# alan-turing-institute/mogp-emulator

Measured on AMD Instinct MI355X. Metric: GP fits/sec (+ fit+grad/s, predict pts/s), 64-output n=2000 d=10 on 1 MI355X, fp64, higher is better.
Workload: dtype f64

## Files before the change

mogp_emulator_amd/csrc/kernels_chol.hip:

```cpp
#include <algorithm>
#include <cstdlib>
#include "launch.h"
#include "chol128_dev.h"

namespace mogp {

typedef double v2d __attribute__((ext_vector_type(2)));
typedef double v4d __attribute__((ext_vector_type(4)));

__device__ __forceinline__ int slot_emu(const int* idx, int z) { return idx ? idx[z] : z; }

template <int RM>
__device__ __forceinline__ void logdet_gram_dev(const BatchView& v, int emu, double* __restrict__ res, double* red) {
  const int ld = v.LD, R = v.R;
  const double* A = v.A + (size_t)emu * v.MS;
  double s = 0.;
  double acc[RM * (RM + 1) / 2];
#pragma unroll
  for (int e = 0; e < RM * (RM + 1) / 2; ++e) acc[e] = 0.;
  for (int i = threadIdx.x; i < v.n; i += 256) {
    s += log(A[(size_t)i * ld + i]);
    double y[RM];
#pragma unroll
    for (int r = 0; r < RM; ++r) y[r] = (r < R) ? A[(size_t)(v.n + r) * ld + i] : 0.0;
// ... 225 lines not shown
      s += part[1][lane];
      s += part[2][lane];
      w[2 * lane] -= s[0];
      w[2 * lane + 1] -= s[1];
    }
    __syncthreads();
  };
  double Lc[64], rdgw = 0.0;
  const int myblk = rg == 0 ? 1 : 0;
  auto preload_diag = [&]() {
    if (rg < 2) {
      const double* Lb = Ld[myblk];
      const double dg = Lb[lane * 65 + lane];
      rdgw = (j0 + 64 * myblk + lane < n) ? 1.0 / dg : 0.0;
#pragma unroll
      for (int j = 0; j < 64; ++j) Lc[j] = Lb[j * 65 + lane];
      __builtin_amdgcn_sched_barrier(0);
#pragma unroll
      for (int j = 0; j < 64; ++j) Lc[j] *= -rdgw;
    }
  };
  auto solve_diag = [&](int blk) {
    const int k0 = j0 + 64 * blk;
    if (rg == (blk ? 0 : 1)) {
      if (!HOIST) preload_diag();
      double bs = w[64 * blk + lane] * rdgw;
      __builtin_amdgcn_sched_barrier(0);
      int xlo = 0, xhi = 0;
#pragma unroll
      for (int j = 63; j >= 0; --j) {
        const int lo = __builtin_amdgcn_readlane(__double2loint(bs), j), hi = __builtin_amdgcn_readlane(__double2hiint(bs), j);
        asm("v_writelane_b32 %0, %1, %2" : "+v"(xlo) : "s"(lo), "n"(j));
        asm("v_writelane_b32 %0, %1, %2" : "+v"(xhi) : "s"(hi), "n"(j));
        bs = __builtin_fma(Lc[j], __hiloint2double(hi, lo), bs);
      }
      double xout = __hiloint2double(xhi, xlo);
      xs[64 * blk + lane] = xout;
      if (__double_as_longlong(xout) == -1ll) xout = __builtin_nan("");
      st_agent(alpha + k0 + lane, xout);
    }
    __syncthreads();
  };
  auto poll_values = [&](int cc, int lo) {
    if (t >= lo && t < lo + 64) {
      const double* p = alpha + 128 * cc + t;
      double x = ld_agent(p);
      int spins = 0;
      while (__double_as_longlong(x) == -1ll && spins++ < spin_limit) {
        __builtin_amdgcn_s_sleep(1);
        x = ld_agent(p);
      }
      if (__double_as_longlong(x) == -1ll) {
        timed_out = 1;
        __hip_atomic_store(status + emu, epoch, __ATOMIC_RELAXED, __HIP_MEMORY_SCOPE_AGENT);
        __builtin_amdgcn_fence(__ATOMIC_RELEASE, "agent");
        x = 0.0;
      }
      xs[t] = x;
    }
    __syncthreads();
  };
  __syncthreads();
  if (HOIST) preload_diag();
  if (res && c == 0) logdet_gram_dev<1>(v, emu, res, red);
  if (nch - 1 > c) {
    load_tile(tA, 128 * (nch - 1) + 64);
    load_tile(tB, 128 * (nch - 1));
  } else {
    load_tile(tA, j0 + 64);
  }
  for (int cc = nch - 1; cc > c; --cc) {
    poll_values(cc, 64);
    apply_tile(tA, 64, 128);
    if (cc - 1 > c) load_tile(tA, 128 * (cc - 1) + 64);
    else load_tile(tA, j0 + 64);
    poll_values(cc, 0);
    apply_tile(tB, 0, 128);
    if (cc - 1 > c) load_tile(tB, 128 * (cc - 1));
  }
  solve_diag(1);
  apply_tile(tA, 64, 64);
  solve_diag(0);
  if (res && c == 0 && t == 0) {
    const int st = info[emu];
    const bool gave_up = timed_out || __hip_atomic_load(status + emu, __ATOMIC_RELAXED, __HIP_MEMORY_SCOPE_AGENT) == epoch;
    int rep = (st == 0 && gave_up) ? BACKSOLVE_TIMEOUT : st;
    if (mc_abort && *mc_abort != 0u) rep = MCHOL_ABORTED;
    res[(size_t)emu * RES_STRIDE + 1] = (double)rep;
  }
}

__global__ __launch_bounds__(256) void combine_rows_kernel(BatchView v, const double* __restrict__ M) {
  const int emu = slot_emu(v.idx, blockIdx.y);
  const int ld = v.LD, R = v.R;
  const int i = blockIdx.x * 256 + threadIdx.x;
  if (i >= ld) return;
  const double* Zb = v.Z + (size_t)emu * R * ld;
  const double* Mb = M + (size_t)emu * (RMAX + 1) * RMAX;
  double z[RMAX];
#pragma unroll
  for (int r = 0; r < RMAX; ++r) z[r] = (r < R) ? Zb[(size_t)r * ld + i] : 0.0;
  for (int c = 0; c < v.RA; ++c) {
    double s = 0.;
#pragma unroll
    for (int r = 0; r < RMAX; ++r) s = __builtin_fma(Mb[c * RMAX + r], z[r], s);
    v.alpha[((size_t)emu * v.RA + c) * ld + i] = s;
  }
}

__global__ __launch_bounds__(256) void alpha_linv_kernel(BatchView v) {
  __shared__ double red[4][128];
  typedef double a2 __attribute__((ext_vector_type(2)));
  const int emu = slot_emu(v.idx, blockIdx.y);
  const int ld = v.LD, n = v.n, R = v.R;
  const double* Li = v.Linv + (size_t)emu * v.MS;
  const int lane = threadIdx.x & 63, wave = threadIdx.x >> 6;
  const int i0 = blockIdx.x * 128, i = i0 + 2 * lane;
  for (int r = 0; r < R; ++r) {
    const double* y = v.A + (size_t)emu * v.MS + (size_t)(n + r) * ld;
    a2 s = {0., 0.};
    if (i0 < n) {
#pragma unroll 16
      for (int k = i0 + wave; k < n; k += 4) {
        const a2 l = *reinterpret_cast<const a2*>(Li + (size_t)k * ld + i);
        const double yk = y[k];
        s[0] = __builtin_fma(l[0], yk, s[0]);
        s[1] = __builtin_fma(l[1], yk, s[1]);
      }
    }
    red[wave][2 * lane] = s[0];
    red[wave][2 * lane + 1] = s[1];
    __syncthreads();
    if (threadIdx.x < 128) {
      const int c = i0 + (int)threadIdx.x, t = threadIdx.x;
      v.Z[((size_t)emu * R + r) * ld + c] = (c < n) ? red[0][t] + red[1][t] + red[2][t] + red[3][t] : 0.0;
    }
    __syncthreads();
  }
}

__global__ __launch_bounds__(256) void loo_variance_kernel(BatchView v, double* __restrict__ out, int out_ld) {
  __shared__ double red[4][64];
  const int emu = slot_emu(v.idx, blockIdx.y);
  const int ld = v.LD, n = v.n;
  const double* Li = v.Linv + (size_t)emu * v.MS;
  const int lane = threadIdx.x & 63, wave = threadIdx.x >> 6;
  const int i0 = blockIdx.x * 64, i = i0 + lane;
  double s = 0.;
#pragma unroll 8
  for (int k = i0 + wave; k < n; k += 4) {
    const double x = Li[(size_t)k * ld + i];
    s = __builtin_fma(x, x, s);
  }
  red[wave][lane] = s;
  __syncthreads();
  if (wave == 0 && i < n) out[(size_t)blockIdx.y * out_ld + i] = fmax(1.0 / (red[0][lane] + red[1][lane] + red[2][lane] + red[3][lane]), 0.0);
}

constexpr int IMPL_MAXRANK = 16;
__global__ __launch_bounds__(256) void implausibility_kernel(int nb, const double* __restrict__ mean, const double* __restrict__ var, int ld,
                                                             int m, const double* __restrict__ prm, int rank, double* __restrict__ out) {
  const int j = blockIdx.x * 256 + threadIdx.x;
  if (j >= m) return;
  double top[IMPL_MAXRANK];
#pragma unroll
  for (int r = 0; r < IMPL_MAXRANK; ++r) top[r] = -1.0;
  for (int k = 0; k < nb; ++k) {
    const double mu = mean[(size_t)k * ld + j] + prm[3 * k + 2];
    const double vv = fmax(var[(size_t)k * ld + j], 0.0) + prm[3 * k + 1];
    double I = fabs(prm[3 * k] - mu) / sqrt(vv);
#pragma unroll
    for (int r = 0; r < IMPL_MAXRANK; ++r)
      if (r <= rank && I > top[r]) {
        const double t = top[r];
        top[r] = I;
        I = t;
      }
  }
  double res = top[0];
#pragma unroll
  for (int r = 1; r < IMPL_MAXRANK; ++r)
    if (r == rank) res = top[r];
  out[j] = res;
}

__global__ __launch_bounds__(256) void implausibility_top_kernel(int nb, const double* __restrict__ mean, const double* __restrict__ var, int ld,
                                                                 int m, const double* __restrict__ prm, int keep, double* __restrict__ out,
                                                                 long out_ld) {
  const int j = blockIdx.x * 256 + threadIdx.x;
  if (j >= m) return;
  double top[IMPL_MAXRANK];
#pragma unroll
  for (int r = 0; r < IMPL_MAXRANK; ++r) top[r] = -INFINITY;
  for (int k = 0; k < nb; ++k) {
    const double mu = mean[(size_t)k * ld + j] + prm[3 * k + 2];
    const double vv = fmax(var[(size_t)k * ld + j], 0.0) + prm[3 * k + 1];
    double I = fabs(prm[3 * k] - mu) / sqrt(vv);
#pragma unroll
    for (int r = 0; r < IMPL_MAXRANK; ++r)
      if (r < keep && I > top[r]) {
        const double t = top[r];
        top[r] = I;
        I = t;
      }
  }
#pragma unroll
  for (int r = 0; r < IMPL_MAXRANK; ++r)
    if (r < keep) out[(size_t)r * out_ld + j] = top[r];
}

__global__ __launch_bounds__(256) void implausibility_merge_kernel(int nparts, const double* __restrict__ lists, long ld, int m, int rank,
                                                                  double* __restrict__ out) {
  const int j = blockIdx.x * 256 + threadIdx.x;
  if (j >= m) return;
  double top[IMPL_MAXRANK];
#pragma unroll
  for (int r = 0; r < IMPL_MAXRANK; ++r) top[r] = -1.0;
  const int keep = rank + 1;
  for (int p = 0; p < nparts; ++p)
    for (int q = 0; q < keep; ++q) {
      double I = lists[((size_t)p * keep + q) * ld + j];
#pragma unroll
      for (int r = 0; r < IMPL_MAXRANK; ++r)
        if (r <= rank && I > top[r]) {
          const double t = top[r];
          top[r] = I;
          I = t;
        }
    }
  double res = top[0];
#pragma unroll
  for (int r = 1; r < IMPL_MAXRANK; ++r)
    if (r == rank) res = top[r];
  out[j] = res;
}

constexpr int MEAN_MAXQ = RMAX;
__device__ __forceinline__ double add_nc(double a, double b) {
#pragma clang fp contract(off)
  return a + b;
}
__device__ __forceinline__ double sub_nc(double a, double b) {
#pragma clang fp contract(off)
  return a - b;
}
__device__ __forceinline__ double mul_nc(double a, double b) {
#pragma clang fp contract(off)
  return a * b;
}
__global__ __launch_bounds__(256) void predict_mean_finish_kernel(int nb, int m, int D, int R, int nbasis, const double* __restrict__ basis,
                                                                  const double* __restrict__ coef, const double* __restrict__ dots,
                                                                  const double* __restrict__ LA, double* __restrict__ mean,
                                                                  double* __restrict__ var, long ld, int nterm,
                                                                  const double* __restrict__ dbasis, const int* __restrict__ ddims,
                                                                  const int* __restrict__ dpowers, double* __restrict__ deriv) {
  const int j = blockIdx.x * 256 + threadIdx.x;
  const int k = blockIdx.y;
  if (j >= m) return;
  const double* c = coef + (size_t)k * nbasis;
  if (mean) {
    if (R == 1) {
      double v = c[0];
      for (int t = 1; t < nbasis; ++t) v = add_nc(v, mul_nc(c[t], basis[(size_t)t * m + j]));
      mean[(size_t)k * ld + j] = add_nc(mean[(size_t)k * ld + j], v);
    } else {
      const int q = R - 1;
      const double* dk = dots + (size_t)k * R * m;
      double mu = dk[j];
      for (int t = 0; t < q; ++t) mu = add_nc(mu, mul_nc(c[t], basis[(size_t)t * m + j]));
      mean[(size_t)k * ld + j] = mu;
      if (var) {
        const double* La = LA + (size_t)k * q * q;
        double rm[MEAN_MAXQ], add = 0.;
#pragma unroll
        for (int t = 0; t < MEAN_MAXQ; ++t) {
          if (t < q) {
            double sres = sub_nc(basis[(size_t)t * m + j], dk[(size_t)(1 + t) * m + j]);
#pragma unroll
            for (int p = 0; p < MEAN_MAXQ; ++p)
              if (p < t) sres = sub_nc(sres, mul_nc(La[t * q + p], rm[p]));
            rm[t] = sres / La[t * q + t];
            add = add_nc(add, mul_nc(rm[t], rm[t]));
          }
        }
        var[(size_t)k * ld + j] = add_nc(var[(size_t)k * ld + j], add);
      }
    }
  }
  if (deriv && nterm > 0) {
    for (int t = 0; t < nterm; ++t) {
      const int d = ddims[t];
      bool first = true;
      for (int u = 0; u < t; ++u) first = first && (ddims[u] != d);
      if (!first) continue;
      double mid = 0.;
      for (int u = t; u < nterm; ++u)
        if (ddims[u] == d) mid = add_nc(mid, mul_nc(mul_nc(c[u + 1], (double)dpowers[u]), dbasis[(size_t)u * m + j]));
      double* o = deriv + ((size_t)k * m + j) * D + d;
      *o = add_nc(*o, mid);
    }
  }
}

__global__ __launch_bounds__(64) void trtri_leaf_kernel(BatchView v, const double* __restrict__ Lmat) {
  __shared__ double Ls[64 * 65];
  const int emu = __builtin_amdgcn_readfirstlane(slot_emu(v.idx, blockIdx.y));
  const int ld = v.LD;
  const int d0 = blockIdx.x * 64;
  const double* __restrict__ L = Lmat + (size_t)emu * v.MS + (size_t)d0 * ld + d0;
  double* Li = v.Linv + (size_t)emu * v.MS;
  const int t = threadIdx.x;
#pragma unroll 8
  for (int r = 0; r < 64; ++r) Ls[r * 65 + t] = L[(size_t)r * ld + t];
  __builtin_amdgcn_wave_barrier();
  double x[64];
#pragma unroll
  for (int c = 0; c < 64; ++c) {
    double s0 = (c == t) ? 1.0 : 0.0, s1 = 0., s2 = 0., s3 = 0.;
#pragma unroll
    for (int p = 0; p < c; ++p) {
      const double lv = Ls[c * 65 + p];
      if ((p & 3) == 0) s0 = __builtin_fma(-x[p], lv, s0);
      else if ((p & 3) == 1) s1 = __builtin_fma(-x[p], lv, s1);
      else if ((p & 3) == 2) s2 = __builtin_fma(-x[p], lv, s2);
      else s3 = __builtin_fma(-x[p], lv, s3);
    }
    x[c] = ((s0 + s1) + (s2 + s3)) / Ls[c * 65 + c];
  }
#pragma unroll
  for (int i = 0; i < 64; ++i) Li[(size_t)(d0 + i) * ld + d0 + t] = x[i];
  if ((blockIdx.x & 1) == 0 && d0 + 64 < ld) {
#pragma unroll 8
    for (int i = 0; i < 64; ++i) Li[(size_t)(d0 + i) * ld + d0 + 64 + t] = 0.0;
  }
}

__global__ void extract_kernel(const double* __restrict__ src, int NP, int n, double* __restrict__ out, int mode) {
  const int j = blockIdx.x * blockDim.x + threadIdx.x;
  const int i = blockIdx.y;
  if (j >= n) return;
  double x;
  if (mode == 0) x = src[(size_t)i * NP + j];
  else if (mode == 1) x = (i <= j) ? src[(size_t)j * NP + i] : 0.0;
  else x = (j <= i) ? src[(size_t)i * NP + j] : src[(size_t)j * NP + i];
  out[(size_t)i * n + j] = x;
}

void launch_logdet(const BatchView& v, const int* info, double* res, hipStream_t s, const int* bs_status, int bs_epoch, const unsigned* mc_abort) {
  hipLaunchKernelGGL(logdet_kernel, dim3(v.nb), dim3(256), 0, s, v, info, res, bs_status, bs_epoch, mc_abort);
}

void launch_combine_rows(const BatchView& v, const double* M, hipStream_t s) {
  hipLaunchKernelGGL(combine_rows_kernel, dim3((v.LD + 255) / 256, v.nb), dim3(256), 0, s, v, M);
}

bool launch_backsolve_chain(const BatchView& v, int epoch, int* status, int n_cu, hipStream_t s, const int* info, double* res, const unsigned* mc_abort) {
  const int nch = (v.n + 127) / 128;
  static const int spin_limit = [] { const char* e = getenv("MOGP_BS_SPIN"); return e ? atoi(e) : (1 << 20); }();
  prof_begin("backsolve", s);
  const bool bound = v.nb * nch <= n_cu;
  double* r = (v.R == 1 && bound) ? res : nullptr;
  if (bound) hipLaunchKernelGGL(backsolve_chain_kernel<true>, dim3(v.nb * nch), dim3(256), 0, s, v, nullptr, epoch, nch, status, spin_limit, info, r, mc_abort);
  else hipLaunchKernelGGL(backsolve_chain_kernel<false>, dim3(v.nb * nch), dim3(256), 0, s, v, nullptr, epoch, nch, status, spin_limit, info, r, mc_abort);
  prof_end("backsolve", s, 0., (double)v.nb * 4.0 * (double)v.n * (double)v.n);
  return r != nullptr;
}

void launch_backsolve(const BatchView& v, hipStream_t s) {
  hipLaunchKernelGGL(backsolve_init_kernel, dim3((v.NP + 255) / 256, v.nb), dim3(256), 0, s, v);
  const int nblk = (v.n + 63) / 64;
  for (int kb = nblk - 1; kb >= 0; --kb) {
    const int k0 = kb * 64;
    const bool fused = v.R == 1;
    if (!fused || kb == nblk - 1) hipLaunchKernelGGL(backsolve_diag_kernel, dim3(v.nb), dim3(64), 0, s, v, k0);
    if (k0 > 0) {
      const dim3 grid((k0 / 2 + BSG_THREADS - 1) / BSG_THREADS, v.nb);
      if (fused) hipLaunchKernelGGL(backsolve_gemv4_kernel<true>, grid, dim3(256), 0, s, v, k0);
      else hipLaunchKernelGGL(backsolve_gemv_kernel<RMAX>, grid, dim3(BSG_THREADS), 0, s, v, k0);
    }
  }
}

void launch_alpha_from_linv(const BatchView& v, hipStream_t s) {
  hipLaunchKernelGGL(alpha_linv_kernel, dim3(v.NP / 128, v.nb), dim3(256), 0, s, v);
}

void launch_loo_variance(const BatchView& v, double* out, int out_ld, hipStream_t s) {
  hipLaunchKernelGGL(loo_variance_kernel, dim3((v.n + 63) / 64, v.nb), dim3(256), 0, s, v, out, out_ld);
}

void launch_implausibility(int nb, const double* mean, const double* var, int ld, int m, const double* prm, int rank, double* out,
                           hipStream_t s) {
  hipLaunchKernelGGL(implausibility_kernel, dim3((m + 255) / 256), dim3(256), 0, s, nb, mean, var, ld, m, prm, rank, out);
}

void launch_implausibility_top(int nb, const double* mean, const double* var, int ld, int m, const double* prm, int keep, double* out,
                               long out_ld, hipStream_t s) {
  hipLaunchKernelGGL(implausibility_top_kernel, dim3((m + 255) / 256), dim3(256), 0, s, nb, mean, var, ld, m, prm, keep, out, out_ld);
}

void launch_implausibility_merge(int nparts, const double* lists, long ld, int m, int rank, double* out, hipStream_t s) {
  hipLaunchKernelGGL(implausibility_merge_kernel, dim3((m + 255) / 256), dim3(256), 0, s, nparts, lists, ld, m, rank, out);
}

__device__ __forceinline__ double int_pow(double x, int p) {
  if (p == 0) return 1.0;
  if (p == 1) return x;
  if (p == 2) return x * x;
  return pow(x, (double)p);
}
__global__ __launch_bounds__(256) void mean_basis_kernel(const double* __restrict__ Xs, int m, int D, int nterm, const int* __restrict__ dims,
                                                         const int* __restrict__ powers, double* __restrict__ basis, double* __restrict__ dbasis) {
  const int j = blockIdx.x * 256 + threadIdx.x;
  if (j >= m) return;
  basis[j] = 1.0;
  for (int t = 0; t < nterm; ++t) {
    const double x = Xs[(size_t)j * D + dims[t]];
    basis[(size_t)(t + 1) * m + j] = int_pow(x, powers[t]);
    dbasis[(size_t)t * m + j] = int_pow(x, powers[t] - 1);
  }
}
void launch_mean_basis(const double* Xs, int m, int D, int nterm, const int* dims, const int* powers, double* basis, double* dbasis, hipStream_t s) {
  hipLaunchKernelGGL(mean_basis_kernel, dim3((m + 255) / 256), dim3(256), 0, s, Xs, m, D, nterm, dims, powers, basis, dbasis);
}

void launch_predict_mean_finish(int nb, int m, int D, int R, int nbasis, const double* basis, const double* coef, const double* dots,
                                const double* LA, double* mean, double* var, long ld, int nterm, const double* dbasis, const int* ddims,
                                const int* dpowers, double* deriv, hipStream_t s) {
  hipLaunchKernelGGL(predict_mean_finish_kernel, dim3((m + 255) / 256, nb), dim3(256), 0, s, nb, m, D, R, nbasis, basis, coef, dots, LA,
                     mean, var, ld, nterm, dbasis, ddims, dpowers, deriv);
}

void launch_trtri_merges(const BatchView& v, hipStream_t s);

void launch_trtri(const BatchView& v, hipStream_t s) {
  hipLaunchKernelGGL(trtri_leaf_kernel, dim3(v.NP / 64, v.nb), dim3(64), 0, s, v, (const double*)v.A);
  launch_trtri_merges(v, s);
}

void launch_extract(const double* src, int NP, int n, double* out, int mode, hipStream_t s) {
  hipLaunchKernelGGL(extract_kernel, dim3((n + 255) / 256, n), dim3(256), 0, s, src, NP, n, out, mode);
}

}
```

mogp_emulator_amd/csrc/kernels_gemm.hip:

```cpp
#include <algorithm>
#include <type_traits>
#include "launch.h"
#include "trsm_dev.h"
#include "gemm_dev.h"
#include "gemm_loop_dev.h"

namespace mogp {



template <int WT>
__global__ __launch_bounds__(256, 2) void update_kernel(BatchView v, int c0, int k0, int k1, int nt, int ntiles) {
  extern __shared__ __attribute__((aligned(16))) double smem[];
  using C = Cfg<WT>;
  int z, tile;
  decode_block(v.nb, ntiles, z, tile);
  if (z >= v.nb) return;
  int ti, tj;
  if (ntiles == nt) {
    ti = tile;
    tj = 0;
  } else {
    ti = (tile + 1) >> 1;
    tj = (tile > 0 && (tile & 1) == 0) ? 1 : 0;
  }
  const int emu = slot_to_emu(v.idx, z);
  double* A = v.A + (size_t)emu * v.MS;
  const int ld = v.LD;
  const int i0 = c0 + ti * C::BM, j0 = c0 + tj * C::BM;
  v4d acc[WT][WT];
  gemm_mainloop<WT, true, true>(A + (size_t)i0 * ld + k0, ld, A + (size_t)j0 * ld + k0, ld, (k1 - k0) / BK, acc, smem);
  for_each_acc<WT>(acc, [&](int r, int c, double x) {
    double* p = A + (size_t)(i0 + r) * ld + (j0 + c);
    *p -= x;
  });
}

__global__ __launch_bounds__(256, 3) void trsm128_lds_kernel(BatchView v, int c0, int r0, const double* __restrict__ Lpack128) {
  extern __shared__ __attribute__((aligned(16))) double smem[];
  const int emu = slot_to_emu(v.idx, blockIdx.y);
  trsm128_lds_dev(v, c0, r0, Lpack128 + (size_t)emu * PACK128_STRIDE, emu, blockIdx.x, smem);
}

template <int WT, int MODE>
__device__ __forceinline__ void merge_mainloop(const double* __restrict__ Ag, int lda, const double* __restrict__ Bg, int ldb, int nk, int nk_full,
                                               v4d (&acc)[WT][WT], double* smem, int wr, int wc) {
  using C = Cfg<WT>;
  const int lane = threadIdx.x & 63;
  const int fr = lane & 15, fk = lane >> 4;
#pragma unroll
  for (int i = 0; i < WT; ++i)
#pragma unroll
    for (int j = 0; j < WT; ++j) acc[i][j] = (v4d){0., 0., 0., 0.};
  if (nk <= 0) return;
  const size_t stepB = (size_t)BK * ldb;
  v2d ra[C::CH], rb[C::CH];
  const unsigned offA = g2r_off<WT, true>(lda), offB = g2r_off<WT, false>(ldb);
  g2r<WT, true>(Ag, lda, offA, ra);
  g2r<WT, false>(Bg, ldb, offB, rb);
  r2s<WT, true>(smem, ra);
  r2s<WT, false>(smem + C::OPSZ, rb);
  __syncthreads();
  auto step = [&](int kt, auto S_, auto E_) {
    constexpr int S = decltype(S_)::value, E = decltype(E_)::value;
    const double* sA = smem + (kt & 1) * 2 * C::OPSZ;
    const double* sB = sA + C::OPSZ;
    const bool more = (kt + 1 < nk);
    if (more) {
      Ag += BK;
      Bg += stepB;
      g2r<WT, true>(Ag, lda, offA, ra);
      g2r<WT, false>(Bg, ldb, offB, rb);
    }
    if (S < WT && E > 0) {
#pragma unroll
      for (int kk = 0; kk < 4; ++kk) {
        double a[WT], b[WT];
        const int k = kk * 4 + fk;
#pragma unroll
        for (int i = S; i < WT; ++i) a[i] = sA[((2 * i + wr) * 16 + fr) * LDK + k];
#pragma unroll
        for (int j = 0; j < E; ++j) b[j] = sB[k * C::LDM + (2 * j + wc) * 16 + fr];
#pragma unroll
        for (int i = S; i < WT; ++i)
#pragma unroll
          for (int j = 0; j < E; ++j) acc[i][j] = __builtin_amdgcn_mfma_f64_16x16x4f64(a[i], b[j], acc[i][j], 0, 0, 0);
      }
    }
    if (more) {
      double* dA = smem + ((kt + 1) & 1) * 2 * C::OPSZ;
      r2s<WT, true>(dA, ra);
      r2s<WT, false>(dA + C::OPSZ, rb);
    }
    __syncthreads();
  };
  using I0 = std::integral_constant<int, 0>;
  using IW = std::integral_constant<int, WT>;
  int kt = 0;
  static_assert(WT == 2 || WT == 4, "phase lists are written for two or four sub-tiles per wave");
  if (MODE == 0) {
    for (const int end = min(nk, wc); kt < end; ++kt) step(kt, I0(), I0());
    for (const int end = min(nk, 2 + wc); kt < end; ++kt) step(kt, I0(), std::integral_constant<int, 1>());
    if (WT == 4) {
      for (const int end = min(nk, 4 + wc); kt < end; ++kt) step(kt, I0(), std::integral_constant<int, 2>());
      for (const int end = min(nk, 6 + wc); kt < end; ++kt) step(kt, I0(), std::integral_constant<int, 3>());
    }
    for (; kt < nk; ++kt) step(kt, I0(), IW());
  } else {
    for (const int end = min(nk, nk_full + wr + 1); kt < end; ++kt) step(kt, I0(), IW());
    for (const int end = min(nk, nk_full + 2 + wr + 1); kt < end; ++kt) step(kt, std::integral_constant<int, 1>(), IW());
    if (WT == 4) {
      for (const int end = min(nk, nk_full + 4 + wr + 1); kt < end; ++kt) step(kt, std::integral_constant<int, 2>(), IW());
      for (const int end = min(nk, nk_full + 6 + wr + 1); kt < end; ++kt) step(kt, std::integral_constant<int, 3>(), IW());
    }
    for (; kt < nk; ++kt) step(kt, IW(), IW());
  }
}

template <int WT, int STEP>
__global__ __launch_bounds__(256, 2) void trtri_merge_kernel(BatchView v, int h, int tiles_per_dim, int nodes) {
  extern __shared__ __attribute__((aligned(16))) double smem[];
  using C = Cfg<WT>;
  const int tpn = tiles_per_dim * tiles_per_dim;
  int z, t;
  decode_block(v.nb, nodes * tpn, z, t);
  if (z >= v.nb) return;
  const int node = t / tpn, bx = t % tpn;
  const int emu = slot_to_emu(v.idx, z);
  const int ld = v.LD;
  const int base = node * 2 * h;
  if (base + h >= v.NP) return;
  const int m2 = min(h, v.NP - base - h);
  int ti, tj;
  if (STEP == 0) {
    tj = bx / tiles_per_dim;
    ti = bx % tiles_per_dim;
  } else {
    ti = tiles_per_dim - 1 - (bx / tiles_per_dim);
    tj = bx % tiles_per_dim;
  }
  const int i0 = ti * C::BM, j0 = tj * C::BM;
  if (i0 >= m2) return;
  const double* L = v.A + (size_t)emu * v.MS;
  double* Li = v.Linv + (size_t)emu * v.MS;
  double* S = v.Kinv + (size_t)emu * v.MS;
  const int lane = threadIdx.x & 63, wave = __builtin_amdgcn_readfirstlane(threadIdx.x >> 6);
  const int wr = wave >> 1, wc = wave & 1;
  v4d acc[WT][WT];
  auto store = [&](double* dst, double sign) {
#pragma unroll
    for (int i = 0; i < WT; ++i)
#pragma unroll
      for (int j = 0; j < WT; ++j)
#pragma unroll
        for (int r = 0; r < 4; ++r)
          dst[(size_t)((2 * i + wr) * 16 + (lane >> 4) + 4 * r) * ld + (2 * j + wc) * 16 + (lane & 15)] = sign * acc[i][j][r];
  };
  if (STEP == 0) {
    const double* Ag = L + (size_t)(base + h + i0) * ld + base + j0;
    const double* Bg = Li + (size_t)(base + j0) * ld + base + j0;
    merge_mainloop<WT, 0>(Ag, ld, Bg, ld, (h - j0) / BK, 0, acc, smem, wr, wc);
    store(S + (size_t)(base + h + i0) * ld + base + j0, 1.0);
  } else {
    const double* Ag = Li + (size_t)(base + h + i0) * ld + base + h;
    const double* Bg = S + (size_t)(base + h) * ld + base + j0;
    const int kend = min(i0 + C::BM, m2);
    merge_mainloop<WT, 1>(Ag, ld, Bg, ld, kend / BK, i0 / BK, acc, smem, wr, wc);
    store(Li + (size_t)(base + h + i0) * ld + base + j0, -1.0);
  }
}

template <int WT, int TRI>
__device__ __forceinline__ void kinv_mainloop(const double* __restrict__ Ag, const double* __restrict__ Bg, int ld, int nk, v4d (&acc)[WT][WT],
                                              double* smem, int wr, int wc) {
  using C = Cfg<WT>;
  const int lane = threadIdx.x & 63;
  const int fr = lane & 15, fk = lane >> 4;
  const size_t stepA = (size_t)BK * ld;
  v2d ra[C::CH], rb[C::CH];
  const unsigned offA = g2r_off<WT, false>(ld);
  g2r<WT, false>(Ag, ld, offA, ra);
  g2r<WT, false>(Bg, ld, offA, rb);
  r2s<WT, false>(smem, ra);
  r2s<WT, false>(smem + C::OPSZ, rb);
  __syncthreads();
  auto step = [&](int kt, auto E_) {
    constexpr int E = decltype(E_)::value;
    const double* sA = smem + (kt & 1) * 2 * C::OPSZ;
    const double* sB = sA + C::OPSZ;
    const bool more = (kt + 1 < nk);
    if (more) {
      Ag += stepA;
      Bg += stepA;
      g2r<WT, false>(Ag, ld, offA, ra);
      g2r<WT, false>(Bg, ld, offA, rb);
    }
    constexpr int JN = (TRI == 0) ? WT : ((TRI == 1) ? E : E - 1);
    if (E > 0 && JN > 0) {
#pragma unroll
      for (int kk = 0; kk < 4; ++kk) {
        double a[WT], b[WT];
        const int k = kk * 4 + fk;
#pragma unroll
        for (int i = 0; i < E; ++i) a[i] = sA[k * C::LDM + (2 * i + wr) * 16 + fr];
#pragma unroll
        for (int j = 0; j < JN; ++j) b[j] = sB[k * C::LDM + (2 * j + wc) * 16 + fr];
#pragma unroll
        for (int i = 0; i < E; ++i)
#pragma unroll
          for (int j = 0; j < JN; ++j)
            if (TRI == 0 || (TRI == 1 && j <= i) || (TRI == 2 && j < i)) acc[i][j] = __builtin_amdgcn_mfma_f64_16x16x4f64(a[i], b[j], acc[i][j], 0, 0, 0);
      }
    }
    if (more) {
      double* dA = smem + ((kt + 1) & 1) * 2 * C::OPSZ;
      r2s<WT, false>(dA, ra);
      r2s<WT, false>(dA + C::OPSZ, rb);
    }
    __syncthreads();
  };
  static_assert(WT == 2 || WT == 4, "phase list written for two or four sub-tiles per wave");
  int kt = 0;
  for (const int end = min(nk, wr); kt < end; ++kt) step(kt, std::integral_constant<int, 0>());
  for (const int end = min(nk, 2 + wr); kt < end; ++kt) step(kt, std::integral_constant<int, 1>());
  if (WT == 4) {
    for (const int end = min(nk, 4 + wr); kt < end; ++kt) step(kt, std::integral_constant<int, 2>());
    for (const int end = min(nk, 6 + wr); kt < end; ++kt) step(kt, std::integral_constant<int, 3>());
  }
  for (; kt < nk; ++kt) step(kt, std::integral_constant<int, WT>());
}

template <int WT>
__global__ __launch_bounds__(256, 2) void kinv_kernel(BatchView v, int ntiles, int kend) {
  extern __shared__ __attribute__((aligned(16))) double smem[];
  using C = Cfg<WT>;
  int z, tile;
  decode_block(v.nb, ntiles, z, tile);
  if (z >= v.nb) return;
  int ti = (int)((sqrt(8.0 * tile + 1.0) - 1.0) * 0.5);
  while (ti * (ti + 1) / 2 > tile) --ti;
  while ((ti + 1) * (ti + 2) / 2 <= tile) ++ti;
  const int tj = tile - ti * (ti + 1) / 2;
  const int emu = slot_to_emu(v.idx, z);
  const int ld = v.LD;
  const double* Li = v.Linv + (size_t)emu * v.MS;
  double* Ki = v.Kinv + (size_t)emu * v.MS;
  const int i0 = ti * C::BM, j0 = tj * C::BM;
  const int lane = threadIdx.x & 63, wave = __builtin_amdgcn_readfirstlane(threadIdx.x >> 6);
  const int wr = wave >> 1, wc = wave & 1;
  v4d acc[WT][WT];
#pragma unroll
  for (int i = 0; i < WT; ++i)
#pragma unroll
    for (int j = 0; j < WT; ++j) acc[i][j] = (v4d){0., 0., 0., 0.};
  const double* Ag = Li + (size_t)i0 * ld + i0;
  const double* Bg = Li + (size_t)i0 * ld + j0;
  const int nk = (kend - i0) / BK;
  if (nk <= 0) return;
  const int tri = (ti != tj) ? 0 : (wr < wc ? 2 : 1);
  if (tri == 0) kinv_mainloop<WT, 0>(Ag, Bg, ld, nk, acc, smem, wr, wc);
  else if (tri == 1) kinv_mainloop<WT, 1>(Ag, Bg, ld, nk, acc, smem, wr, wc);
  else kinv_mainloop<WT, 2>(Ag, Bg, ld, nk, acc, smem, wr, wc);
#pragma unroll
  for (int i = 0; i < WT; ++i)
#pragma unroll
    for (int j = 0; j < WT; ++j) {
      if (tri == 0 || (tri == 1 && j <= i) || (tri == 2 && j < i)) {
#pragma unroll
        for (int r = 0; r < 4; ++r)
          Ki[(size_t)(i0 + (2 * i + wr) * 16 + (lane >> 4) + 4 * r) * ld + j0 + (2 * j + wc) * 16 + (lane & 15)] = acc[i][j][r];
      }
    }
}

__global__ __launch_bounds__(256, 2) void predict_v_store_kernel(BatchView v, const double* __restrict__ Ks, int MP, int nti, int ntj,
                                                               double* __restrict__ Vout) {
  extern __shared__ __attribute__((aligned(16))) double smem[];
  using C = Cfg<4>;
  const int npairs = (nti + 1) / 2;
  const int nsr = (npairs + 3) / 4, nsc = (ntj + 15) / 16;
  int z, tile;
  decode_block(v.nb, nsr * nsc * 64, z, tile);
  if (z >= v.nb) return;
  const int st = tile >> 6, w = tile & 63;
  const int pr = (st / nsc) * 4 + (w >> 4), tj = (st % nsc) * 16 + (w & 15);
  if (pr >= npairs || tj >= ntj) return;
  const int emu = slot_to_emu(v.idx, z);
  const int ld = v.LD;
  const double* Li = v.Linv + (size_t)emu * v.MS;
  const double* K = Ks + (size_t)z * MP * ld;
  const int j0 = tj * C::BM;
  const int ti_long = nti - 1 - pr, ti_short = pr;
  double* V = Vout + (size_t)z * v.NP * MP;
  for (int pass = 0; pass < 2; ++pass) {
    if (pass == 1 && ti_short == ti_long) break;
    const int ti = pass == 0 ? ti_long : ti_short;
    const int i0 = ti * C::BM;
    v4d acc[4][4];
    gemm_mainloop<4, true, true>(Li + (size_t)i0 * ld, ld, K + (size_t)j0 * ld, ld, (i0 + C::BM) / BK, acc, smem);
    for_each_acc<4>(acc, [&](int r, int c, double x) { V[(size_t)(i0 + r) * MP + j0 + c] = x; });
  }
}

__global__ __launch_bounds__(512, 4) void update_tri8_kernel(BatchView v, int c0, int k0, int k1, int ntiles) {
  extern __shared__ __attribute__((aligned(16))) double smem[];
  using C = WCfg<128, 128, 2, 4>;
  int z, tile;
  decode_block(v.nb, ntiles, z, tile);
  if (z >= v.nb) return;
  int ti = (int)((sqrt(8.0 * tile + 1.0) - 1.0) * 0.5);
  while (ti * (ti + 1) / 2 > tile) --ti;
  while ((ti + 1) * (ti + 2) / 2 <= tile) ++ti;
  const int tj = tile - ti * (ti + 1) / 2;
  const int emu = slot_to_emu(v.idx, z);
  double* A = v.A + (size_t)emu * v.MS;
  const int ld = v.LD;
  const int i0 = c0 + ti * 128, j0 = c0 + tj * 128;
  v4d acc[C::TI][C::TJ];
  mainloop_w<128, 128, 2, 4>(A + (size_t)i0 * ld + k0, ld, A + (size_t)j0 * ld + k0, ld, (k1 - k0) / BK, acc, smem);
  for_each_acc_w<4>(acc, [&](int r, int c, double x) {
    double* p = A + (size_t)(i0 + r) * ld + (j0 + c);
    *p -= x;
  });
}

constexpr bool PV_SWZ = true;
constexpr int PVW_LGC = 3, PVW_SC = 1 << PVW_LGC, PVW_SR = 64 >> PVW_LGC;
template <int WR, int WC, bool TRI>
__global__ __launch_bounds__(64 * WR * WC, (WR * WC >= 8 ? 4 : 2)) void predict_var_w_kernel(
    BatchView v, const double* __restrict__ Ks, int MP, int nti, int ntj, double* __restrict__ partial) {
  extern __shared__ __attribute__((aligned(16))) double smem[];
  using C = WCfg<128, 128, WR, WC>;
  const int npairs = (nti + 1) / 2;
  constexpr int lgc = PVW_LGC, SC = PVW_SC, SR = PVW_SR;
  const int nsr = (npairs + SR - 1) / SR, nsc = (ntj + SC - 1) / SC;
  const int t = threadIdx.x, lane = t & 63, wave = TRI ? __builtin_amdgcn_readfirstlane(t >> 6) : (t >> 6);
  const int wr = wave / WC, wc = wave % WC;
  int z, tile;
  decode_block(v.nb, nsr * nsc * 64, z, tile);
  if (z >= v.nb) return;
  const int st = tile >> 6, w = tile & 63;
  const int pr = (st / nsc) * SR + (w >> lgc), tj = (st % nsc) * SC + (w & (SC - 1));
  if (pr >= npairs || tj >= ntj) return;
  const int emu = slot_to_emu(v.idx, z);
  const int ld = v.LD;
  const double* Li = v.Linv + (size_t)emu * v.MS;
  const double* K = Ks + (size_t)z * MP * ld;
  const int j0 = tj * 128;
  const int ti_long = nti - 1 - pr, ti_short = pr;
  for (int pass = 0; pass < 2; ++pass) {
    if (pass == 1 && ti_short == ti_long) break;
    const int ti = pass == 0 ? ti_long : ti_short;
    const int i0 = ti * 128;
    v4d acc[C::TI][C::TJ];
    const int nk = TRI ? min(i0 + 128, (v.n + 15) & ~15) / BK : (i0 + 128) / BK;
    mainloop_w<128, 128, WR, WC, TRI, true, PV_SWZ>(Li + (size_t)i0 * ld, ld, K + (size_t)j0 * ld, ld, nk, acc, smem, i0 / BK, v.n - i0);
    double* red = smem;
#pragma unroll
    for (int j = 0; j < C::TJ; ++j) {
      double s = 0.;
#pragma unroll
      for (int i = 0; i < C::TI; ++i)
#pragma unroll
        for (int r = 0; r < 4; ++r) s += acc[i][j][r] * acc[i][j][r];
      s += __shfl_xor(s, 16);
      s += __shfl_xor(s, 32);
      if (lane < 16) red[wr * 128 + wc * 16 * C::TJ + j * 16 + lane] = s;
    }
    __syncthreads();
    if (t < 128) {
      double s = 0.;
#pragma unroll
      for (int q = 0; q < WR; ++q) s += red[q * 128 + t];
      partial[((size_t)z * nti + ti) * MP + j0 + t] = s;
    }
    __syncthreads();
  }
}

__global__ __launch_bounds__(256, 2) void fullcov_kernel(BatchView v, const double* __restrict__ V, int MP, int m, int ntiles, int kend,
                                                       double* __restrict__ cov) {
  extern __shared__ __attribute__((aligned(16))) double smem[];
  using C = Cfg<4>;
  int z, tile;
  decode_block(v.nb, ntiles, z, tile);
  if (z >= v.nb) return;
  int ti = (int)((sqrt(8.0 * tile + 1.0) - 1.0) * 0.5);
  while (ti * (ti + 1) / 2 > tile) --ti;
  while ((ti + 1) * (ti + 2) / 2 <= tile) ++ti;
  const int tj = tile - ti * (ti + 1) / 2;
  const double* Vz = V + (size_t)z * v.NP * MP;
  double* Cz = cov + (size_t)z * m * m;
  const int i0 = ti * C::BM, j0 = tj * C::BM;
  v4d acc[4][4];
  gemm_mainloop<4, false, false>(Vz + i0, MP, Vz + j0, MP, kend / BK, acc, smem);
  for_each_acc<4>(acc, [&](int r, int c, double x) {
    const int i = i0 + r, j = j0 + c;
    if (i < m && j < m) {
      const double val = Cz[(size_t)i * m + j] - x;
      Cz[(size_t)i * m + j] = val;
      if (ti != tj) Cz[(size_t)j * m + i] = val;
    }
  });
}

__global__ void predict_var_finish_kernel(BatchView v, const double* __restrict__ partial, int m, int MP, int nti, double* var, int var_ld) {
  const int z = blockIdx.y;
  const int j = blockIdx.x * blockDim.x + threadIdx.x;
  if (j >= m) return;
  const int emu = slot_to_emu(v.idx, z);
  double s = 0.;
  for (int t = 0; t < nti; ++t) s += partial[((size_t)z * nti + t) * MP + j];
  var[(size_t)z * var_ld + j] = v.P[(size_t)emu * v.PS + v.D] - s;
}

template <int WT>
static constexpr size_t smem_bytes() { return Cfg<WT>::SMEM_DOUBLES * sizeof(double); }

static int padded_grid(int nb, int ntiles) { return ((nb & 7) == 0) ? nb * ntiles : nb * ntiles; }

void launch_update_narrow(const BatchView& v, int c0, int k0, int k1, hipStream_t s) {
  const int nt = (v.NP - c0) / 64;
  if (nt <= 0) return;
  hipLaunchKernelGGL((update_kernel<2>), dim3(padded_grid(v.nb, nt)), dim3(256), smem_bytes<2>(), s, v, c0, k0, k1, nt, nt);
}

void launch_update_narrow_pair(const BatchView& v, int c0, int k0, int k1, hipStream_t s) {
  const int nt = (v.NP - c0) / 64;
  if (nt <= 0) return;
  const int ntiles = std::max(1, 2 * nt - 1);
  const double m = (double)(v.NP - c0);
  prof_begin("chol_update", s);
  hipLaunchKernelGGL((update_kernel<2>), dim3(padded_grid(v.nb, ntiles)), dim3(256), smem_bytes<2>(), s, v, c0, k0, k1, nt, ntiles);
  prof_end("chol_update", s, (double)v.nb * (m * 128.0 - 128.0 * 128.0 / 2.0) * 2.0 * (k1 - k0), (double)v.nb * (16.0 * m * 128.0 + 8.0 * (m + 128.0) * (k1 - k0)));
}

void launch_update_wide(const BatchView& v, int c0, int k0, int k1, hipStream_t s) {
  const int nt = (v.NP - c0) / 128;
  if (nt <= 0) return;
  const double m = (double)(v.NP - c0);
  prof_begin("chol_update", s);
  hipLaunchKernelGGL((update_kernel<4>), dim3(padded_grid(v.nb, nt)), dim3(256), smem_bytes<4>(), s, v, c0, k0, k1, nt, nt);
  prof_end("chol_update", s, (double)v.nb * (m * 128.0 - 128.0 * 128.0 / 2.0) * 2.0 * (k1 - k0), (double)v.nb * (16.0 * m * 128.0 + 8.0 * (m + 128.0) * (k1 - k0)));
}

void launch_update_trailing(const BatchView& v, int c0, int k0, int k1, hipStream_t s) {
  const int nt = (v.NP - c0) / 128;
  if (nt <= 0) return;
  const int ntiles = nt * (nt + 1) / 2;
  const double m = (double)(v.NP - c0);
  prof_begin("syrk_trailing", s);
  hipLaunchKernelGGL(update_tri8_kernel, dim3(padded_grid(v.nb, ntiles)), dim3(512), smem_bytes<4>(), s, v, c0, k0, k1, ntiles);
  prof_end("syrk_trailing", s, (double)v.nb * m * m * (k1 - k0), (double)v.nb * (8.0 * m * m + 8.0 * m * (k1 - k0)));
}

void launch_trtri_merges(const BatchView& v, hipStream_t s) {
  const double alg = ((double)v.n / v.NP) * ((double)v.n / v.NP) * ((double)v.n / v.NP);
  for (int h = 64; h < v.NP; h *= 2) {
    const int nodes = (v.NP + 2 * h - 1) / (2 * h);
    double fl = 0.;
    for (int q = 0; q < nodes; ++q) {
      const double m2 = std::min<double>(h, (double)v.NP - (double)q * 2 * h - h);
      if (m2 > 0) fl += m2 * h * (double)h + m2 * m2 * h;
    }
    if (h > 64) prof_begin("trtri_merge", s);
    const long wide_tiles = (long)v.nb * nodes * (h / 128) * (h / 128);
    if (h >= 512 && wide_tiles >= 3000) {
      const int tpd = h / 128;
      hipLaunchKernelGGL((trtri_merge_kernel<4, 0>), dim3(padded_grid(v.nb, tpd * tpd * nodes)), dim3(256), smem_bytes<4>(), s, v, h, tpd, nodes);
      hipLaunchKernelGGL((trtri_merge_kernel<4, 1>), dim3(padded_grid(v.nb, tpd * tpd * nodes)), dim3(256), smem_bytes<4>(), s, v, h, tpd, nodes);
    } else {
      const int tpd = h / 64;
      hipLaunchKernelGGL((trtri_merge_kernel<2, 0>), dim3(padded_grid(v.nb, tpd * tpd * nodes)), dim3(256), smem_bytes<2>(), s, v, h, tpd, nodes);
      hipLaunchKernelGGL((trtri_merge_kernel<2, 1>), dim3(padded_grid(v.nb, tpd * tpd * nodes)), dim3(256), smem_bytes<2>(), s, v, h, tpd, nodes);
    }
    if (h > 64) prof_end("trtri_merge", s, (double)v.nb * fl * alg, 0.);
  }
}

constexpr int PVQ_LGC = 4, PVQ_SC = 1 << PVQ_LGC, PVQ_SR = 64 >> PVQ_LGC;
template <bool TRI>
__global__ __launch_bounds__(256, 2) void predict_var_q_kernel(BatchView v, const double* __restrict__ Ks, int MP, int nti, int ntj,
                                                               double* __restrict__ partial) {
  extern __shared__ __attribute__((aligned(16))) double smem[];
  using C = WCfg<128, 64, 2, 2>;
  constexpr int lgc = PVQ_LGC, SC = PVQ_SC, SR = PVQ_SR;
  const int nsr = (nti + SR - 1) / SR, nsc = (ntj + SC - 1) / SC;
  const int t = threadIdx.x, lane = t & 63, wave = __builtin_amdgcn_readfirstlane(t >> 6);
  const int wr = wave / 2, wc = wave % 2;
  int z, tile;
  decode_block(v.nb, nsr * nsc * 64, z, tile);
  if (z >= v.nb) return;
  const int st = tile >> 6, w = tile & 63;
  const int pr = (st / nsc) * SR + (w >> lgc), tj = (st % nsc) * SC + (w & (SC - 1));
  if (pr >= nti || tj >= ntj) return;
  const int emu = slot_to_emu(v.idx, z);
  const int ld = v.LD;
  const double* Li = v.Linv + (size_t)emu * v.MS;
  const double* K = Ks + (size_t)z * MP * ld;
  const int j0 = tj * 64;
  const int ti = nti - 1 - pr;
  const int i0 = ti * 128;
  v4d acc[C::TI][C::TJ];
  const int nk = min(i0 + 128, (v.n + 15) & ~15) / BK;
  mainloop_qt<128, 64, 2, 2>(Li + (size_t)i0 * ld, ld, K + (size_t)j0 * ld, ld, nk, acc, smem, TRI ? i0 / BK : nk, TRI ? v.n - i0 : 128);
  double* red = smem;
#pragma unroll
  for (int j = 0; j < C::TJ; ++j) {
    double s = 0.;
#pragma unroll
    for (int i = 0; i < C::TI; ++i)
#pragma unroll
      for (int r = 0; r < 4; ++r) s += acc[i][j][r] * acc[i][j][r];
    s += __shfl_xor(s, 16);
    s += __shfl_xor(s, 32);
    if (lane < 16) red[wr * 64 + wc * 16 * C::TJ + j * 16 + lane] = s;
  }
  __syncthreads();
  if (t < 64) partial[((size_t)z * nti + ti) * MP + j0 + t] = red[t] + red[64 + t];
}

void launch_kinv(const BatchView& v, int n_cu, hipStream_t s) {
  const int kend = ((v.n + 15) / 16) * 16;
  const int nt = (v.n + 127) / 128;
  const int ntiles = nt * (nt + 1) / 2;
  const bool small = (long)v.nb * ntiles < 2L * 2 * n_cu;
  prof_begin("kinv", s);
  if (small) {
    const int nt2 = (v.n + 63) / 64;
    const int ntiles2 = nt2 * (nt2 + 1) / 2;
    hipLaunchKernelGGL(kinv_kernel<2>, dim3(padded_grid(v.nb, ntiles2)), dim3(256), smem_bytes<2>(), s, v, ntiles2, kend);
  } else
    hipLaunchKernelGGL(kinv_kernel<4>, dim3(padded_grid(v.nb, ntiles)), dim3(256), smem_bytes<4>(), s, v, ntiles, kend);
  prof_end("kinv", s, (double)v.nb * (double)v.n * v.n * v.n / 3.0, 0.);
}

void launch_predict_var(const BatchView& v, const double* Ks, int m, int MP, double* partial, double* var, int var_ld, int n_cu, hipStream_t s) {
  const int nti = (v.n + 127) / 128, ntj = MP / 128;
  prof_begin("predict_var", s);
  const long pair_tasks = (long)v.nb * ((nti + 1) / 2) * ntj;
  if (pair_tasks < 2L * 2 * n_cu) {
    const int ntq = MP / 64;
    constexpr size_t lds_q = (size_t)QCfg<128, 64>::SMEM_DOUBLES * sizeof(double);
    const int nsq = ((nti + PVQ_SR - 1) / PVQ_SR) * ((ntq + PVQ_SC - 1) / PVQ_SC);
    hipLaunchKernelGGL((predict_var_q_kernel<true>), dim3(padded_grid(v.nb, nsq * 64)), dim3(256), lds_q, s, v, Ks, MP, nti, ntq, partial);
  } else {
    const int nst = (((nti + 1) / 2 + PVW_SR - 1) / PVW_SR) * ((ntj + PVW_SC - 1) / PVW_SC);
    hipLaunchKernelGGL((predict_var_w_kernel<2, 4, true>), dim3(padded_grid(v.nb, nst * 64)), dim3(512), smem_bytes<4>(), s, v, Ks, MP, nti, ntj, partial);
  }
  prof_end("predict_var", s, (double)v.nb * (double)m * v.n * v.n, 0.);
  hipLaunchKernelGGL(predict_var_finish_kernel, dim3((m + 255) / 256, v.nb), dim3(256), 0, s, v, partial, m, MP, nti, var, var_ld);
}

void launch_trsm128(const BatchView& v, int c0, const double* Lpack128, hipStream_t s) {
  const int rows = v.NP - c0 - 128;
  if (rows <= 0) return;
  prof_begin("chol_trsm128", s);
  hipLaunchKernelGGL(trsm128_lds_kernel, dim3(rows / 64, v.nb), dim3(256), TRSM128L_LDS * sizeof(double), s, v, c0, c0 + 128, Lpack128);
  prof_end("chol_trsm128", s, (double)v.nb * rows * 128.0 * 128.0, (double)v.nb * 2.0 * 8.0 * rows * 128.0);
}

void launch_predict_v_store(const BatchView& v, const double* Ks, int m, int MP, double* V, hipStream_t s) {
  const int nti = (v.n + 127) / 128, ntj = MP / 128;
  const int nsup = (((nti + 1) / 2 + 3) / 4) * ((ntj + 15) / 16) * 64;
  prof_begin("predict_var", s);
  hipLaunchKernelGGL(predict_v_store_kernel, dim3(padded_grid(v.nb, nsup)), dim3(256), smem_bytes<4>(), s, v, Ks, MP, nti, ntj, V);
  prof_end("predict_var", s, (double)v.nb * (double)m * v.n * v.n, 0.);
}

void launch_predict_fullcov(const BatchView& v, const double* Ks, int m, int MP, double* V, double* cov, hipStream_t s) {
  launch_predict_v_store(v, Ks, m, MP, V, s);
  const int ntj = MP / 128;
  const int ntiles = ntj * (ntj + 1) / 2;
  const int kend = ((v.n + 15) / 16) * 16;
  prof_begin("fullcov_syrk", s);
  hipLaunchKernelGGL(fullcov_kernel, dim3(padded_grid(v.nb, ntiles)), dim3(256), smem_bytes<4>(), s, v, V, MP, m, ntiles, kend, cov);
  prof_end("fullcov_syrk", s, (double)v.nb * (double)m * m * v.n, 0.);
}

}
```

Before: 16870.

## Fuse trtri leaf inversion and first two merge levels into one block kernel

Replaces the separate 64x64 leaf-inversion kernel and the h=64 and h=128 merge launches with a single 256-wide block kernel. In it, four waves each invert one diagonal leaf using packed-triangular LDS staging, then run the two lowest merge levels in place with workgroup barriers. This removes several small kernel launches and their global round trips for the triangular inverse. The cost is lower parallelism per launch and serialized merge tiles inside one workgroup.

```diff
diff --git a/mogp_emulator_amd/csrc/kernels_chol.hip b/mogp_emulator_amd/csrc/kernels_chol.hip
--- a/mogp_emulator_amd/csrc/kernels_chol.hip
+++ b/mogp_emulator_amd/csrc/kernels_chol.hip
@@ -551,39 +551,6 @@
   }
 }
 
-__global__ __launch_bounds__(64) void trtri_leaf_kernel(BatchView v, const double* __restrict__ Lmat) {
-  __shared__ double Ls[64 * 65];
-  const int emu = __builtin_amdgcn_readfirstlane(slot_emu(v.idx, blockIdx.y));
-  const int ld = v.LD;
-  const int d0 = blockIdx.x * 64;
-  const double* __restrict__ L = Lmat + (size_t)emu * v.MS + (size_t)d0 * ld + d0;
-  double* Li = v.Linv + (size_t)emu * v.MS;
-  const int t = threadIdx.x;
-#pragma unroll 8
-  for (int r = 0; r < 64; ++r) Ls[r * 65 + t] = L[(size_t)r * ld + t];
-  __builtin_amdgcn_wave_barrier();
-  double x[64];
-#pragma unroll
-  for (int c = 0; c < 64; ++c) {
-    double s0 = (c == t) ? 1.0 : 0.0, s1 = 0., s2 = 0., s3 = 0.;
-#pragma unroll
-    for (int p = 0; p < c; ++p) {
-      const double lv = Ls[c * 65 + p];
-      if ((p & 3) == 0) s0 = __builtin_fma(-x[p], lv, s0);
-      else if ((p & 3) == 1) s1 = __builtin_fma(-x[p], lv, s1);
-      else if ((p & 3) == 2) s2 = __builtin_fma(-x[p], lv, s2);
-      else s3 = __builtin_fma(-x[p], lv, s3);
-    }
-    x[c] = ((s0 + s1) + (s2 + s3)) / Ls[c * 65 + c];
-  }
-#pragma unroll
-  for (int i = 0; i < 64; ++i) Li[(size_t)(d0 + i) * ld + d0 + t] = x[i];
-  if ((blockIdx.x & 1) == 0 && d0 + 64 < ld) {
-#pragma unroll 8
-    for (int i = 0; i < 64; ++i) Li[(size_t)(d0 + i) * ld + d0 + 64 + t] = 0.0;
-  }
-}
-
 __global__ void extract_kernel(const double* __restrict__ src, int NP, int n, double* __restrict__ out, int mode) {
   const int j = blockIdx.x * blockDim.x + threadIdx.x;
   const int i = blockIdx.y;
@@ -682,10 +649,7 @@
 
 void launch_trtri_merges(const BatchView& v, hipStream_t s);
 
-void launch_trtri(const BatchView& v, hipStream_t s) {
-  hipLaunchKernelGGL(trtri_leaf_kernel, dim3(v.NP / 64, v.nb), dim3(64), 0, s, v, (const double*)v.A);
-  launch_trtri_merges(v, s);
-}
+void launch_trtri(const BatchView& v, hipStream_t s) { launch_trtri_merges(v, s); }
 
 void launch_extract(const double* src, int NP, int n, double* out, int mode, hipStream_t s) {
   hipLaunchKernelGGL(extract_kernel, dim3((n + 255) / 256, n), dim3(256), 0, s, src, NP, n, out, mode);
diff --git a/mogp_emulator_amd/csrc/kernels_gemm.hip b/mogp_emulator_amd/csrc/kernels_gemm.hip
--- a/mogp_emulator_amd/csrc/kernels_gemm.hip
+++ b/mogp_emulator_amd/csrc/kernels_gemm.hip
@@ -4,6 +4,7 @@
 #include "trsm_dev.h"
 #include "gemm_dev.h"
 #include "gemm_loop_dev.h"
+#include "trtri_plan.h"
 
 namespace mogp {
 
@@ -118,32 +119,10 @@
 }
 
 template <int WT, int STEP>
-__global__ __launch_bounds__(256, 2) void trtri_merge_kernel(BatchView v, int h, int tiles_per_dim, int nodes) {
-  extern __shared__ __attribute__((aligned(16))) double smem[];
+__device__ __forceinline__ void trtri_merge_tile(const double* L, double* Li, double* S, int ld, int base, int h, int m2, int ti, int tj,
+                                                 double* smem) {
   using C = Cfg<WT>;
-  const int tpn = tiles_per_dim * tiles_per_dim;
-  int z, t;
-  decode_block(v.nb, nodes * tpn, z, t);
-  if (z >= v.nb) return;
-  const int node = t / tpn, bx = t % tpn;
-  const int emu = slot_to_emu(v.idx, z);
-  const int ld = v.LD;
-  const int base = node * 2 * h;
-  if (base + h >= v.NP) return;
-  const int m2 = min(h, v.NP - base - h);
-  int ti, tj;
-  if (STEP == 0) {
-    tj = bx / tiles_per_dim;
-    ti = bx % tiles_per_dim;
-  } else {
-    ti = tiles_per_dim - 1 - (bx / tiles_per_dim);
-    tj = bx % tiles_per_dim;
-  }
   const int i0 = ti * C::BM, j0 = tj * C::BM;
-  if (i0 >= m2) return;
-  const double* L = v.A + (size_t)emu * v.MS;
-  double* Li = v.Linv + (size_t)emu * v.MS;
-  double* S = v.Kinv + (size_t)emu * v.MS;
   const int lane = threadIdx.x & 63, wave = __builtin_amdgcn_readfirstlane(threadIdx.x >> 6);
   const int wr = wave >> 1, wc = wave & 1;
   v4d acc[WT][WT];
@@ -168,6 +147,99 @@
     merge_mainloop<WT, 1>(Ag, ld, Bg, ld, kend / BK, i0 / BK, acc, smem, wr, wc);
     store(Li + (size_t)(base + h + i0) * ld + base + j0, -1.0);
   }
+}
+
+template <int WT, int STEP>
+__global__ __launch_bounds__(256, 2) void trtri_merge_kernel(BatchView v, int h, int tiles_per_dim, int nodes) {
+  extern __shared__ __attribute__((aligned(16))) double smem[];
+  using C = Cfg<WT>;
+  const int tpn = tiles_per_dim * tiles_per_dim;
+  int z, t;
+  decode_block(v.nb, nodes * tpn, z, t);
+  if (z >= v.nb) return;
+  const int node = t / tpn, bx = t % tpn;
+  const int emu = slot_to_emu(v.idx, z);
+  const int ld = v.LD;
+  const int base = node * 2 * h;
+  if (base + h >= v.NP) return;
+  const int m2 = min(h, v.NP - base - h);
+  int ti, tj;
+  if (STEP == 0) {
+    tj = bx / tiles_per_dim;
+    ti = bx % tiles_per_dim;
+  } else {
+    ti = tiles_per_dim - 1 - (bx / tiles_per_dim);
+    tj = bx % tiles_per_dim;
+  }
+  if (ti * C::BM >= m2) return;
+  trtri_merge_tile<WT, STEP>(v.A + (size_t)emu * v.MS, v.Linv + (size_t)emu * v.MS, v.Kinv + (size_t)emu * v.MS, ld, base, h, m2, ti, tj, smem);
+}
+
+constexpr int TRTRI_LEAF_LDS = TRTRI_LEAF * (TRTRI_LEAF + 1) / 2;
+constexpr int TRTRI_BLOCK_LDS = (TRTRI_BLOCK / TRTRI_LEAF) * TRTRI_LEAF_LDS;
+static_assert(TRTRI_BLOCK_LDS >= Cfg<2>::SMEM_DOUBLES, "the merge loop's buffers alias the leaf staging");
+static_assert(2 * TRTRI_BLOCK_LDS * sizeof(double) <= 160 * 1024, "two workgroups per CU");
+
+__device__ __forceinline__ void trtri_leaf_wave(const double* __restrict__ L, double* Li, int ld, int d0, bool zero_right, double* Ls) {
+  const int t = threadIdx.x & 63;
+  L += (size_t)d0 * ld + d0;
+#pragma unroll 16
+  for (int r = 0; r < 64; ++r)
+    if (t <= r) Ls[r * (r + 1) / 2 + t] = L[(size_t)r * ld + t];
+  __builtin_amdgcn_wave_barrier();
+  double x[64];
+#pragma unroll
+  for (int c = 0; c < 64; ++c) {
+    double s0 = (c == t) ? 1.0 : 0.0, s1 = 0., s2 = 0., s3 = 0.;
+#pragma unroll
+    for (int p = 0; p < c; ++p) {
+      const double lv = Ls[c * (c + 1) / 2 + p];
+      if ((p & 3) == 0) s0 = __builtin_fma(-x[p], lv, s0);
+      else if ((p & 3) == 1) s1 = __builtin_fma(-x[p], lv, s1);
+      else if ((p & 3) == 2) s2 = __builtin_fma(-x[p], lv, s2);
+      else s3 = __builtin_fma(-x[p], lv, s3);
+    }
+    x[c] = ((s0 + s1) + (s2 + s3)) / Ls[c * (c + 1) / 2 + c];
+  }
+#pragma unroll
+  for (int i = 0; i < 64; ++i) Li[(size_t)(d0 + i) * ld + d0 + t] = x[i];
+  if (zero_right) {
+#pragma unroll 8
+    for (int i = 0; i < 64; ++i) Li[(size_t)(d0 + i) * ld + d0 + 64 + t] = 0.0;
+  }
+}
+
+__global__ __launch_bounds__(256, 2) void trtri_block_kernel(BatchView v, int nblk) {
+  extern __shared__ __attribute__((aligned(16))) double smem[];
+  int z, b;
+  decode_block(v.nb, nblk, z, b);
+  if (z >= v.nb) return;
+  const int emu = __builtin_amdgcn_readfirstlane(slot_to_emu(v.idx, z));
+  const int ld = v.LD;
+  const double* L = v.A + (size_t)emu * v.MS;
+  double* Li = v.Linv + (size_t)emu * v.MS;
+  double* S = v.Kinv + (size_t)emu * v.MS;
+  const int d0 = b * TRTRI_BLOCK;
+  const int w = trtri_block_width(v.NP, b);
+  const int wave = __builtin_amdgcn_readfirstlane(threadIdx.x >> 6);
+  if (wave * TRTRI_LEAF < w) {
+    const int l0 = d0 + wave * TRTRI_LEAF;
+    trtri_leaf_wave(L, Li, ld, l0, (wave & 1) == 0 && l0 + TRTRI_LEAF < ld, smem + wave * TRTRI_LEAF_LDS);
+  }
+  __syncthreads();
+  const TrtriNodeRange n64 = trtri_block_nodes(v.NP, b, 64);
+#pragma unroll 1
+  for (int q = n64.first; q < n64.first + n64.count; ++q) trtri_merge_tile<2, 0>(L, Li, S, ld, q * 128, 64, 64, 0, 0, smem);
+  __syncthreads();
+#pragma unroll 1
+  for (int q = n64.first; q < n64.first + n64.count; ++q) trtri_merge_tile<2, 1>(L, Li, S, ld, q * 128, 64, 64, 0, 0, smem);
+  if (trtri_block_nodes(v.NP, b, 128).count == 0) return;
+  __syncthreads();
+#pragma unroll 1
+  for (int bx = 0; bx < 4; ++bx) trtri_merge_tile<2, 0>(L, Li, S, ld, d0, 128, 128, bx % 2, bx / 2, smem);
+  __syncthreads();
+#pragma unroll 1
+  for (int bx = 0; bx < 4; ++bx) trtri_merge_tile<2, 1>(L, Li, S, ld, d0, 128, 128, 1 - bx / 2, bx % 2, smem);
 }
 
 template <int WT, int TRI>
@@ -456,14 +528,14 @@
 
 void launch_trtri_merges(const BatchView& v, hipStream_t s) {
   const double alg = ((double)v.n / v.NP) * ((double)v.n / v.NP) * ((double)v.n / v.NP);
-  for (int h = 64; h < v.NP; h *= 2) {
-    const int nodes = (v.NP + 2 * h - 1) / (2 * h);
-    double fl = 0.;
-    for (int q = 0; q < nodes; ++q) {
-      const double m2 = std::min<double>(h, (double)v.NP - (double)q * 2 * h - h);
-      if (m2 > 0) fl += m2 * h * (double)h + m2 * m2 * h;
-    }
-    if (h > 64) prof_begin("trtri_merge", s);
+  const int nblk = trtri_blocks(v.NP);
+  prof_begin("trtri_merge", s);
+  hipLaunchKernelGGL(trtri_block_kernel, dim3(padded_grid(v.nb, nblk)), dim3(256), TRTRI_BLOCK_LDS * sizeof(double), s, v, nblk);
+  prof_end("trtri_merge", s, (double)v.nb * trtri_block_flops(v.NP) * alg, 0.);
+  for (int h = trtri_first_level(); h < v.NP; h *= 2) {
+    const int nodes = trtri_level_nodes(v.NP, h);
+    const double fl = trtri_level_flops(v.NP, h);
+    prof_begin("trtri_merge", s);
     const long wide_tiles = (long)v.nb * nodes * (h / 128) * (h / 128);
     if (h >= 512 && wide_tiles >= 3000) {
       const int tpd = h / 128;
@@ -474,7 +546,7 @@
       hipLaunchKernelGGL((trtri_merge_kernel<2, 0>), dim3(padded_grid(v.nb, tpd * tpd * nodes)), dim3(256), smem_bytes<2>(), s, v, h, tpd, nodes);
       hipLaunchKernelGGL((trtri_merge_kernel<2, 1>), dim3(padded_grid(v.nb, tpd * tpd * nodes)), dim3(256), smem_bytes<2>(), s, v, h, tpd, nodes);
     }
-    if (h > 64) prof_end("trtri_merge", s, (double)v.nb * fl * alg, 0.);
+    prof_end("trtri_merge", s, (double)v.nb * fl * alg, 0.);
   }
 }
 
diff --git a/mogp_emulator_amd/csrc/trtri_plan.h b/mogp_emulator_amd/csrc/trtri_plan.h
--- /dev/null
+++ b/mogp_emulator_amd/csrc/trtri_plan.h
@@ -0,0 +1,38 @@
+#pragma once
+
+namespace mogp {
+
+constexpr int TRTRI_LEAF = 64;
+constexpr int TRTRI_BLOCK = 256;
+
+constexpr int trtri_blocks(int NP) { return (NP + TRTRI_BLOCK - 1) / TRTRI_BLOCK; }
+constexpr int trtri_block_width(int NP, int b) { return NP - b * TRTRI_BLOCK < TRTRI_BLOCK ? NP - b * TRTRI_BLOCK : TRTRI_BLOCK; }
+constexpr int trtri_first_level() { return TRTRI_BLOCK; }
+
+constexpr int trtri_level_nodes(int NP, int h) { return (NP + 2 * h - 1) / (2 * h); }
+constexpr int trtri_node_rows(int NP, int h, int q) { return NP - q * 2 * h - h < h ? NP - q * 2 * h - h : h; }
+
+struct TrtriNodeRange {
+  int first, count;
+};
+constexpr TrtriNodeRange trtri_block_nodes(int NP, int b, int h) {
+  return (h >= trtri_first_level() || 2 * h > trtri_block_width(NP, b)) ? TrtriNodeRange{0, 0}
+                                                                        : TrtriNodeRange{b * (TRTRI_BLOCK / (2 * h)), trtri_block_width(NP, b) / (2 * h)};
+}
+
+constexpr double trtri_leaf_flops() { return (double)TRTRI_LEAF * TRTRI_LEAF * TRTRI_LEAF / 3.0; }
+inline double trtri_level_flops(int NP, int h) {
+  double fl = 0.;
+  for (int q = 0; q < trtri_level_nodes(NP, h); ++q) {
+    const double m2 = (double)trtri_node_rows(NP, h, q);
+    if (m2 > 0) fl += m2 * h * (double)h + m2 * m2 * h;
+  }
+  return fl;
+}
+inline double trtri_block_flops(int NP) {
+  double fl = (double)(NP / TRTRI_LEAF) * trtri_leaf_flops();
+  for (int h = TRTRI_LEAF; h < trtri_first_level() && h < NP; h *= 2) fl += trtri_level_flops(NP, h);
+  return fl;
+}
+
+}
```

Result: no change. 16870 (median of 3 runs) (-0.0%).
